# ParsaEsmati/SEA

Measured on AMD Instinct MI355X. Metric: rollout steps/sec (full-context forward, recompute mode) on cylinder_flow-shaped fields, higher is better.
Workload: dtype bf16

## Files before the change

### sea_amd/csrc/mlp_block.hip

```cpp
#include "gemm_core.hpp"
#include <stdlib.h>

struct MlpBlockLaunch {
    SeaMlpGroup g1[SEA_MAX_MLP_GROUPS];
    SeaMlp2Group g2[SEA_MAX_MLP_GROUPS];
    int tile_start[SEA_MAX_MLP_GROUPS + 1];
    int xcd_start[SEA_MAX_MLP_GROUPS + 1];
    int n_groups;
    float eps;
    int per_xcd;
    int probe;
};

__device__ __forceinline__ void glds16_blk(const void* gsrc, unsigned lds_addr) {
    unsigned keep;
    asm volatile("s_mov_b32 %0, m0\n\ts_mov_b32 m0, %2\n\ts_nop 0\n\tglobal_load_lds_dwordx4 %1, off\n\ts_mov_b32 m0, %0"
                 : "=&s"(keep) : "v"(gsrc), "s"(lds_addr) : "memory");
}

__device__ __forceinline__ void glds16_blk_s(const void* ubase, unsigned lane_off, unsigned lds_addr) {
    unsigned keep;
    asm volatile("s_mov_b32 %0, m0\n\ts_mov_b32 m0, %3\n\ts_nop 0\n\tglobal_load_lds_dwordx4 %1, %2\n\ts_mov_b32 m0, %0"
                 : "=&s"(keep) : "v"(lane_off), "s"(ubase), "s"(lds_addr) : "memory");
}

template <int KT, int NSB>
struct MlpBlockCfg {
    static constexpr int BM = 32, BKB = 128, NS = 4, NW = 8;
    static constexpr int E = KT * 64, S = NSB * 128;
    static constexpr int A_BYTES = KT * BM * BKB, STAGE = KT * 64 * BKB;
    static constexpr int PRM_OFF = A_BYTES + NS * STAGE;
    static constexpr int P1_BYTES = PRM_OFF + 2 * S * 4;
    static constexpr int SLAB_PITCH = 128 * 4 + 16, SLAB = BM * SLAB_PITCH;
    static constexpr int X3_OFF = NW * SLAB;
    static constexpr int RED2_OFF = X3_OFF + KT * BM * BKB;
    static constexpr int P2_BYTES = RED2_OFF + 2 * NW * BM * 4;
    static constexpr int RS = KT == 4 ? 8 : 4, SLOT = 16 * 128;
    static constexpr int RING_OFF = KT == 4 ? A_BYTES : P1_BYTES;
    static constexpr int RING_END = RING_OFF + NW * RS * SLOT;
    static constexpr int BYTES_ = P1_BYTES > P2_BYTES ? P1_BYTES : P2_BYTES;
    static constexpr int BYTES = BYTES_ > RING_END ? BYTES_ : RING_END;
};

__device__ __forceinline__ f32x4 mma16_first(const uint4& a, const uint4& b) {
    return __builtin_amdgcn_mfma_f32_16x16x32_bf16(__builtin_bit_cast(bf16x8, a), __builtin_bit_cast(bf16x8, b), f32x4{0.f, 0.f, 0.f, 0.f}, 0, 0, 0);
}

__device__ __forceinline__ constexpr int blk_col_base(int t, int half, int wq) { return (t >> 1) * 512 + half * 256 + wq * 64 + (t & 1) * 32; }

template <int KT, int NSB>
__global__ __launch_bounds__(512) void mlp_block_kernel(const MlpBlockLaunch L) {
    using T = __bf16;
    using Cf = MlpBlockCfg<KT, NSB>;
    constexpr int BM = 32, BKB = 128, BK = 64, NS = 4, NW = 8;
    constexpr int E = Cf::E, S = Cf::S, NSTAGE = S / 64, NT = NSB / 2;
    constexpr int A_BYTES = Cf::A_BYTES, STAGE = Cf::STAGE;
    constexpr int LPS = KT * 8 / NW;
    constexpr int PRM_OFF = Cf::PRM_OFF;
    constexpr int B1_OFF = 0, RED_OFF = S * 4;
    static_assert(RED_OFF + 2 * NW * BM * 4 <= A_BYTES && (S / 256) * 1024 <= A_BYTES && LPS * NW == KT * 8 && NT % 2 == 0 && Cf::BYTES <= 160 * 1024, "LDS layout of sea_mlp_block");
    static_assert((NT / 2) * 512 == S, "blk_col_base covers the hidden columns once");
    extern __shared__ __attribute__((aligned(16))) char smem[];
    int tile, gi = 0;
    if (L.per_xcd < 0) {
        const int xcd = (int)(blockIdx.x & 7), idx = (int)(blockIdx.x >> 3);
        if (xcd >= L.xcd_start[L.n_groups]) return;
        while (gi + 1 < L.n_groups && xcd >= L.xcd_start[gi + 1]) ++gi;
        tile = L.tile_start[gi] + (xcd - L.xcd_start[gi]) * 32 + idx;
        if (tile >= L.tile_start[gi + 1]) return;
    } else {
        tile = L.per_xcd > 0 ? (int)(blockIdx.x & 7) * L.per_xcd + (int)(blockIdx.x >> 3) : (int)blockIdx.x;
        if (tile >= L.tile_start[L.n_groups]) return;
        while (gi + 1 < L.n_groups && tile >= L.tile_start[gi + 1]) ++gi;
    }
    const SeaMlpGroup& G = L.g1[gi];
    const SeaMlp2Group& H = L.g2[gi];
    const int m0 = (tile - L.tile_start[gi]) * BM, M = G.M;
    const int tid = threadIdx.x, lane = tid & 63;
    const int wave = __builtin_amdgcn_readfirstlane(tid >> 6);
    const int r = lane & 15, g = lane >> 4;
    const int half = wave >> 2, wq = wave & 3;
    const T* A = static_cast<const T*>(G.A);
    const T* W = static_cast<const T*>(G.W1);
    const unsigned lds_base = __builtin_amdgcn_readfirstlane((unsigned)(uintptr_t)smem);
    const int rl = lane >> 3;
    const int chunk = (lane & 7) ^ (rl & 7);
    for (int p = wave; p < 2 * (S / 256); p += NW) {
        const float* src = p < S / 256 ? G.lnw : G.lnb;
        const int q = p < S / 256 ? p : p - S / 256;
        glds16_blk(src + q * 256 + lane * 4, lds_base + (unsigned)(PRM_OFF + p * 1024));
    }
    for (int p = wave; G.X32 == nullptr && p < KT * (BM / 8); p += NW) {
        const int kt = p / (BM / 8), u = p - kt * (BM / 8);
        int row = m0 + u * 8 + rl;
        row = row < M ? row : M - 1;
        glds16_blk(A + (int64_t)row * G.lda + kt * BK + chunk * 8, lds_base + (unsigned)(kt * BM * BKB + u * 8 * BKB));
    }
    const unsigned w1_lane = (unsigned)(((8 * (rl >> 2) + (rl & 3)) * G.ldw + chunk * 8) * 2);
    auto dma_stage = [&](int s) {
        const unsigned base = lds_base + (unsigned)(A_BYTES + (s % NS) * STAGE);
        const int t = s >> 2, u = (s >> 1) & 1, hs = s & 1;
#pragma unroll
        for (int i = 0; i < LPS; ++i) {
            const int p = i * NW + wave;
            const int kt = p >> 3, u8 = p & 7;
            const int urow = blk_col_base(t, hs, u8 >> 1) + 16 * (u8 & 1) + 4 * u;
            glds16_blk_s(W + (int64_t)urow * G.ldw + kt * BK, w1_lane, base + (unsigned)(kt * 64 * BKB + u8 * 8 * BKB));
        }
    };
    dma_stage(0);
    if (G.X32 != nullptr) {
        constexpr int CPT = E / 16;
        const int prow = tid >> 4, pl = tid & 15;
        int row = m0 + prow;
        row = row < M ? row : M - 1;
        const int c0 = pl * CPT;
        float xv[CPT];
#pragma unroll
        for (int c = 0; c < CPT; c += 4) load4(G.X32 + (int64_t)row * G.ldx32 + c0 + c, *reinterpret_cast<float(*)[4]>(xv + c));
        if (G.addend != nullptr) {
#pragma unroll
            for (int c = 0; c < CPT; c += 4) {
                float av[4];
                load4(G.addend + (int64_t)row * G.ldadd + c0 + c, av);
#pragma unroll
                for (int e = 0; e < 4; ++e) xv[c + e] += av[e];
            }
        }
        float gq[CPT], bq[CPT];
#pragma unroll
        for (int c = 0; c < CPT; c += 4) {
            load4(G.gamma + c0 + c, *reinterpret_cast<float(*)[4]>(gq + c));
#pragma unroll
            for (int e = 0; e < 4; ++e) bq[c + e] = 0.f;
            if (G.beta != nullptr) load4(G.beta + c0 + c, *reinterpret_cast<float(*)[4]>(bq + c));
            if (G.mod != nullptr) {
                float mw[4], mb[4];
                const T* mod = static_cast<const T*>(G.mod) + (int64_t)row * G.ldmod;
                load4(mod + c0 + c, mw);
                load4(mod + E + c0 + c, mb);
#pragma unroll
                for (int e = 0; e < 4; ++e) {
                    gq[c + e] += 1.0f + mw[e];
                    bq[c + e] += mb[e];
                }
            }
        }
        float s4[4] = {0.f, 0.f, 0.f, 0.f};
#pragma unroll
        for (int c = 0; c < CPT; c += 4)
#pragma unroll
            for (int e = 0; e < 4; ++e) s4[e] = add1(s4[e], xv[c + e]);
        float sm_ = add1(add1(s4[0], s4[1]), add1(s4[2], s4[3]));
#pragma unroll
        for (int o = 8; o >= 1; o >>= 1) sm_ += __shfl_xor(sm_, o);
        const float mean = sm_ * (1.0f / (float)E);
        float q4[4] = {0.f, 0.f, 0.f, 0.f};
#pragma unroll
        for (int c = 0; c < CPT; c += 4)
#pragma unroll
            for (int e = 0; e < 4; ++e) {
                const float d_ = xv[c + e] - mean;
                q4[e] = fma1(d_, d_, q4[e]);
            }
        float sq = add1(add1(q4[0], q4[1]), add1(q4[2], q4[3]));
#pragma unroll
        for (int o = 8; o >= 1; o >>= 1) sq += __shfl_xor(sq, o);
        const float rstd = 1.0f / sqrtf(sq * (1.0f / (float)E) + G.norm_eps);
#pragma unroll
        for (int c = 0; c < CPT; c += 8) {
            const int col = c0 + c, kt = col >> 6, ck = (col & 63) >> 3;
            bf16x8 pv;
#pragma unroll
            for (int e = 0; e < 8; ++e) pv[e] = (__bf16)((xv[c + e] - mean) * rstd * gq[c + e] + bq[c + e]);
            *reinterpret_cast<bf16x8*>(smem + kt * BM * BKB + prow * BKB + ((ck ^ (prow & 7)) << 4)) = pv;
        }
        asm volatile("s_waitcnt vmcnt(0) lgkmcnt(0)" ::: "memory");
    }
    for (int s = 1; s < NS - 1; ++s) dma_stage(s);

    const T* W2 = static_cast<const T*>(H.W2);
    const unsigned w2_lane = (unsigned)((rl * H.ldw2 + chunk * 8) * 2);
    const T* Wp = static_cast<const T*>(H.Wproj);
    const unsigned wp_lane = (unsigned)((rl * H.ldwp + chunk * 8) * 2);
    constexpr int NSLOT = (E / 16) * (NT / 2);
    constexpr int NJ = E / NW / 16;
    constexpr int NX = NJ * KT;
    auto w2_slot = [&](int k) {
        const unsigned dst = lds_base + (unsigned)(Cf::RING_OFF + (wave * Cf::RS + (k % Cf::RS)) * Cf::SLOT);
        if (k < NSLOT) {
            const int tau = k / (E / 16), j = k - tau * (E / 16);
            const T* ub = W2 + (int64_t)(j * 16) * H.ldw2 + blk_col_base(2 * tau, half, wq);
#pragma unroll
            for (int u = 0; u < 2; ++u)
                glds16_blk_s(ub + (int64_t)(8 * u) * H.ldw2, w2_lane, dst + (unsigned)(u * 1024));
        } else {
            const int kk = k - NSLOT, j = kk / KT, kt = kk - j * KT;
            const T* ub = Wp + (int64_t)(wave * (E / NW) + j * 16) * H.ldwp + kt * BK;
#pragma unroll
            for (int u = 0; u < 2; ++u)
                glds16_blk_s(ub + (int64_t)(8 * u) * H.ldwp, wp_lane, dst + (unsigned)(u * 1024));
        }
    };
    uint4 hid[NT][2];
    float mean[2], rstd[2];
    {
        f32x4 acc[NSB][2];
        uint4 areg[KT][2][2];
#pragma unroll
        for (int i = 0; i < NSB; ++i) {
            acc[i][0] = f32x4{0.f, 0.f, 0.f, 0.f};
            acc[i][1] = f32x4{0.f, 0.f, 0.f, 0.f};
        }
#pragma unroll
        for (int s = 0; s < NSTAGE; ++s) {
            if (s + 2 < NSTAGE) asm volatile("s_waitcnt vmcnt(%0) lgkmcnt(0)" ::"n"(2 * LPS) : "memory");
            else if (s + 1 < NSTAGE) asm volatile("s_waitcnt vmcnt(%0) lgkmcnt(0)" ::"n"(LPS) : "memory");
            else asm volatile("s_waitcnt vmcnt(0) lgkmcnt(0)" ::: "memory");
            __builtin_amdgcn_s_barrier();
            if (s + NS - 1 < NSTAGE) dma_stage(s + NS - 1);
            if (s == 0) {
                const char* sA = smem + r * BKB;
#pragma unroll
                for (int kt = 0; kt < KT; ++kt)
#pragma unroll
                    for (int kc = 0; kc < 2; ++kc) {
                        const int off = ((kc * 4 + g) ^ (r & 7)) << 4;
                        areg[kt][kc][0] = *reinterpret_cast<const uint4*>(sA + kt * BM * BKB + off);
                        areg[kt][kc][1] = *reinterpret_cast<const uint4*>(sA + kt * BM * BKB + 16 * BKB + off);
                    }
                asm volatile("s_waitcnt lgkmcnt(0)" ::: "memory");
            }
            if (s == 1)
                for (int p = wave; p < S / 256; p += NW) glds16_blk(G.b1 + p * 256 + lane * 4, lds_base + (unsigned)(B1_OFF + p * 1024));
            if ((s & 1) == half) {
                const char* sW = smem + A_BYTES + (s % NS) * STAGE + (wq * 16 + r) * BKB;
#pragma unroll
                for (int kt = 0; kt < KT; ++kt)
#pragma unroll
                    for (int kc = 0; kc < 2; ++kc) {
                        const int off = ((kc * 4 + g) ^ (r & 7)) << 4;
                        const uint4 wf = *reinterpret_cast<const uint4*>(sW + kt * 64 * BKB + off);
                        mma16<T>(wf, areg[kt][kc][0], acc[s >> 1][0]);
                        mma16<T>(wf, areg[kt][kc][1], acc[s >> 1][1]);
                    }
            }
        }
        if (L.probe == 1) return;
        float* red = reinterpret_cast<float*>(smem + RED_OFF);
        const float* pb1 = reinterpret_cast<const float*>(smem + B1_OFF);
        const float* pgm = reinterpret_cast<const float*>(smem + PRM_OFF);
        const float* pbt = pgm + S;
        const float inv_s = 1.0f / (float)S;
        float sum[2] = {0.f, 0.f};
#pragma unroll
        for (int i = 0; i < NSB; ++i) {
            const int n = blk_col_base(i >> 1, half, wq) + 8 * g + 4 * (i & 1);
            float bv[4];
            load4(pb1 + n, bv);
#pragma unroll
            for (int mb = 0; mb < 2; ++mb) {
#pragma unroll
                for (int q = 0; q < 4; ++q) acc[i][mb][q] += bv[q];
                sum[mb] += (acc[i][mb][0] + acc[i][mb][1]) + (acc[i][mb][2] + acc[i][mb][3]);
            }
        }
#pragma unroll
        for (int mb = 0; mb < 2; ++mb) {
            sum[mb] += __shfl_xor(sum[mb], 16);
            sum[mb] += __shfl_xor(sum[mb], 32);
            if (g == 0) red[wave * 32 + mb * 16 + r] = sum[mb];
        }
        __syncthreads();
#pragma unroll
        for (int k = 0; k < Cf::RS - 1; ++k) w2_slot(k);
        float sq[2] = {0.f, 0.f};
#pragma unroll
        for (int mb = 0; mb < 2; ++mb) {
            float t = 0.f;
#pragma unroll
            for (int w = 0; w < NW; ++w) t += red[w * 32 + mb * 16 + r];
            mean[mb] = t * inv_s;
        }
#pragma unroll
        for (int i = 0; i < NSB; ++i)
#pragma unroll
            for (int mb = 0; mb < 2; ++mb)
#pragma unroll
                for (int q = 0; q < 4; ++q) {
                    const float c = acc[i][mb][q] - mean[mb];
                    sq[mb] += c * c;
                }
#pragma unroll
        for (int mb = 0; mb < 2; ++mb) {
            sq[mb] += __shfl_xor(sq[mb], 16);
            sq[mb] += __shfl_xor(sq[mb], 32);
            if (g == 0) red[256 + wave * 32 + mb * 16 + r] = sq[mb];
        }
        asm volatile("s_waitcnt lgkmcnt(0)" ::: "memory");
        __builtin_amdgcn_s_barrier();
#pragma unroll
        for (int mb = 0; mb < 2; ++mb) {
            float t = 0.f;
#pragma unroll
            for (int w = 0; w < NW; ++w) t += red[256 + w * 32 + mb * 16 + r];
            rstd[mb] = 1.0f / sqrtf(t * inv_s + L.eps);
        }
#pragma unroll
        for (int i = 0; i < NSB; ++i) {
            const int n = blk_col_base(i >> 1, half, wq) + 8 * g + 4 * (i & 1);
            float gm[4], bt[4];
            load4(pgm + n, gm);
            load4(pbt + n, bt);
#pragma unroll
            for (int mb = 0; mb < 2; ++mb) {
                bf16x4 y;
#pragma unroll
                for (int q = 0; q < 4; ++q) y[q] = (__bf16)gelu_erf_bf16((acc[i][mb][q] - mean[mb]) * rstd[mb] * gm[q] + bt[q]);
                uint2 y2 = *reinterpret_cast<const uint2*>(&y);
                asm volatile("" : "+v"(y2.x), "+v"(y2.y));
                if (i & 1) {
                    hid[i >> 1][mb].z = y2.x;
                    hid[i >> 1][mb].w = y2.y;
                } else {
                    hid[i >> 1][mb].x = y2.x;
                    hid[i >> 1][mb].y = y2.y;
                }
            }
            __builtin_amdgcn_sched_barrier(0);
        }
    }
    __builtin_amdgcn_sched_barrier(0);
    if (L.probe == 2) {
        asm volatile("s_waitcnt vmcnt(0)" ::: "memory");
        return;
    }

    constexpr int NJB = E / 16;
    constexpr int NTOT = NSLOT + NX;
    f32x4 acc2[2][NJB];
    uint4 wp[KT * 2][NJ];
#pragma unroll
    for (int k = 0; k < NTOT; ++k) {
        const int tau = k / NJB, j = k - tau * NJB;
        {
            constexpr int AFTER_MAX = Cf::RS - 2;
            const int after = NTOT - 1 - k < AFTER_MAX ? NTOT - 1 - k : AFTER_MAX;
            switch (after) {
                case 6: asm volatile("s_waitcnt vmcnt(12) lgkmcnt(0)" ::: "memory"); break;
                case 5: asm volatile("s_waitcnt vmcnt(10) lgkmcnt(0)" ::: "memory"); break;
                case 4: asm volatile("s_waitcnt vmcnt(8) lgkmcnt(0)" ::: "memory"); break;
                case 3: asm volatile("s_waitcnt vmcnt(6) lgkmcnt(0)" ::: "memory"); break;
                case 2: asm volatile("s_waitcnt vmcnt(4) lgkmcnt(0)" ::: "memory"); break;
                case 1: asm volatile("s_waitcnt vmcnt(2) lgkmcnt(0)" ::: "memory"); break;
                default: asm volatile("s_waitcnt vmcnt(0) lgkmcnt(0)" ::: "memory"); break;
            }
        }
        if (k + Cf::RS - 1 < NTOT) w2_slot(k + Cf::RS - 1);
        const char* sl = smem + Cf::RING_OFF + (wave * Cf::RS + (k % Cf::RS)) * Cf::SLOT + r * 128;
        if (k >= NSLOT) {
            const int kk = k - NSLOT, jp = kk / KT, kt = kk - jp * KT;
#pragma unroll
            for (int kc = 0; kc < 2; ++kc) wp[kt * 2 + kc][jp] = *reinterpret_cast<const uint4*>(sl + (((kc * 4 + g) ^ (r & 7)) << 4));
            continue;
        }
#pragma unroll
        for (int u2 = 0; u2 < 2; ++u2) {
            const uint4 w = *reinterpret_cast<const uint4*>(sl + (((u2 * 4 + g) ^ (r & 7)) << 4));
            const int t = 2 * tau + u2;
            if (t == 0) {
                acc2[0][j] = mma16_first(w, hid[0][0]);
                acc2[1][j] = mma16_first(w, hid[0][1]);
            } else {
                mma16<T>(w, hid[t][0], acc2[0][j]);
                mma16<T>(w, hid[t][1], acc2[1][j]);
            }
        }
        __builtin_amdgcn_sched_barrier(0);
    }
    __syncthreads();
    if (L.probe == 3) return;
    {
    int tid_l = threadIdx.x;
    asm volatile("" : "+v"(tid_l));
    const int tid = tid_l, lane = tid & 63, r = lane & 15, g = lane >> 4;
    (void)lane;
    constexpr int NH = E / 128, JH = 8;
    const int srow = tid >> 4, scb = (tid & 15) * 8;
    float resv[NH][8];
    {
        int row = m0 + srow;
        row = row < M ? row : M - 1;
#pragma unroll
        for (int h = 0; h < NH; ++h) {
            const int col = h * 128 + scb;
            float b2a[4], b2b[4];
            load4(H.b2 + col, b2a);
            load4(H.b2 + col + 4, b2b);
            float ra[4], rb[4];
            if (H.R != nullptr) {
                load4(H.R + (int64_t)row * H.ldr + col, ra);
                load4(H.R + (int64_t)row * H.ldr + col + 4, rb);
            } else {
                load4(G.X32 + (int64_t)row * G.ldx32 + col, ra);
                load4(G.X32 + (int64_t)row * G.ldx32 + col + 4, rb);
                if (G.addend != nullptr) {
                    float aa[4], ab[4];
                    load4(G.addend + (int64_t)row * G.ldadd + col, aa);
                    load4(G.addend + (int64_t)row * G.ldadd + col + 4, ab);
#pragma unroll
                    for (int q = 0; q < 4; ++q) {
                        ra[q] += aa[q];
                        rb[q] += ab[q];
                    }
                }
            }
#pragma unroll
            for (int q = 0; q < 4; ++q) {
                resv[h][q] = b2a[q] + ra[q];
                resv[h][4 + q] = b2b[q] + rb[q];
            }
        }
    }
    constexpr int CPT = E / 16;
    const int ec0 = (tid & 15) * CPT;
    float ebp[CPT], egq[CPT], ebq[CPT];
    const bool has_norm = H.gamma != nullptr;
#pragma unroll
    for (int h = 0; h < NH; ++h) {
        char* slab = smem + wave * Cf::SLAB;
#pragma unroll
        for (int mb = 0; mb < 2; ++mb)
#pragma unroll
            for (int j = 0; j < JH; ++j)
                *reinterpret_cast<f32x4*>(slab + (mb * 16 + r) * Cf::SLAB_PITCH + (j * 16 + g * 4) * 4) = acc2[mb][h * JH + j];
        if (h == NH - 1) {
            __builtin_amdgcn_sched_barrier(0);
            int m = m0 + srow;
            m = m < M ? m : M - 1;
#pragma unroll
            for (int c = 0; c < CPT; c += 4) {
                load4(H.bproj + ec0 + c, *reinterpret_cast<float(*)[4]>(ebp + c));
#pragma unroll
                for (int q = 0; q < 4; ++q) egq[c + q] = ebq[c + q] = 0.f;
                if (has_norm) {
                    load4(H.gamma + ec0 + c, *reinterpret_cast<float(*)[4]>(egq + c));
                    if (H.beta != nullptr) load4(H.beta + ec0 + c, *reinterpret_cast<float(*)[4]>(ebq + c));
                    if (H.mod != nullptr) {
                        float mw[4], mb[4];
                        const T* mod = static_cast<const T*>(H.mod) + (int64_t)m * H.ldmod;
                        load4(mod + ec0 + c, mw);
                        load4(mod + E + ec0 + c, mb);
#pragma unroll
                        for (int q = 0; q < 4; ++q) {
                            egq[c + q] += 1.0f + mw[q];
                            ebq[c + q] += mb[q];
                        }
                    }
                }
            }
        }
        asm volatile("s_waitcnt lgkmcnt(0)" ::: "memory");
        __builtin_amdgcn_s_barrier();
        {
            float v[8];
#pragma unroll
            for (int q = 0; q < 8; ++q) v[q] = resv[h][q];
#pragma unroll
            for (int w = 0; w < NW; ++w) {
                const float4 a = *reinterpret_cast<const float4*>(smem + w * Cf::SLAB + srow * Cf::SLAB_PITCH + scb * 4);
                const float4 b = *reinterpret_cast<const float4*>(smem + w * Cf::SLAB + srow * Cf::SLAB_PITCH + scb * 4 + 16);
                v[0] += a.x; v[1] += a.y; v[2] += a.z; v[3] += a.w;
                v[4] += b.x; v[5] += b.y; v[6] += b.z; v[7] += b.w;
            }
            const int col = h * 128 + scb, kt = col >> 6, ck = (col & 63) >> 3;
            bf16x8 pv;
#pragma unroll
            for (int q = 0; q < 8; ++q) pv[q] = (__bf16)v[q];
            *reinterpret_cast<bf16x8*>(smem + Cf::X3_OFF + kt * BM * BKB + srow * BKB + ((ck ^ (srow & 7)) << 4)) = pv;
        }
        asm volatile("s_waitcnt lgkmcnt(0)" ::: "memory");
        __builtin_amdgcn_s_barrier();
        if (L.probe == 5 + h) return;
    }

    if (L.probe == 4) return;
    f32x4 acc3[2][NJ];
    {
        const char* sA = smem + Cf::X3_OFF + r * BKB;
#pragma unroll
        for (int kt = 0; kt < KT; ++kt)
#pragma unroll
            for (int kc = 0; kc < 2; ++kc) {
                const int off = ((kc * 4 + g) ^ (r & 7)) << 4;
                const uint4 af0 = *reinterpret_cast<const uint4*>(sA + kt * BM * BKB + off);
                const uint4 af1 = *reinterpret_cast<const uint4*>(sA + kt * BM * BKB + 16 * BKB + off);
#pragma unroll
                for (int j = 0; j < NJ; ++j) {
                    if (kt == 0 && kc == 0) {
                        acc3[0][j] = mma16_first(wp[0][j], af0);
                        acc3[1][j] = mma16_first(wp[0][j], af1);
                    } else {
                        mma16<T>(wp[kt * 2 + kc][j], af0, acc3[0][j]);
                        mma16<T>(wp[kt * 2 + kc][j], af1, acc3[1][j]);
                    }
                }
            }
    }
    constexpr int SEG = 80, YP = (E / 16) * SEG + 16;
    static_assert(BM * YP <= Cf::X3_OFF, "the y tile lies in front of the x3 tile");
#pragma unroll
    for (int i = 0; i < 2; ++i)
#pragma unroll
        for (int j = 0; j < NJ; ++j) {
            const int n = wave * (E / NW) + j * 16 + g * 4;
            *reinterpret_cast<f32x4*>(smem + (i * 16 + r) * YP + (n >> 4) * SEG + (n & 15) * 4) = acc3[i][j];
        }
    asm volatile("s_waitcnt lgkmcnt(0)" ::: "memory");
    __builtin_amdgcn_s_barrier();
    {
        float v[CPT];
#pragma unroll
        for (int c = 0; c < CPT; c += 4) {
            const float4 y = *reinterpret_cast<const float4*>(smem + srow * YP + ((ec0 + c) >> 4) * SEG + ((ec0 + c) & 15) * 4);
            v[c] = y.x + ebp[c]; v[c + 1] = y.y + ebp[c + 1]; v[c + 2] = y.z + ebp[c + 2]; v[c + 3] = y.w + ebp[c + 3];
        }
        if (has_norm) {
            float s4[4] = {0.f, 0.f, 0.f, 0.f};
#pragma unroll
            for (int c = 0; c < CPT; c += 4)
#pragma unroll
                for (int e = 0; e < 4; ++e) s4[e] = add1(s4[e], v[c + e]);
            float sm_ = add1(add1(s4[0], s4[1]), add1(s4[2], s4[3]));
#pragma unroll
            for (int o = 8; o >= 1; o >>= 1) sm_ += __shfl_xor(sm_, o);
            const float mean2 = sm_ * (1.0f / (float)E);
            float q4[4] = {0.f, 0.f, 0.f, 0.f};
#pragma unroll
            for (int c = 0; c < CPT; c += 4)
#pragma unroll
                for (int e = 0; e < 4; ++e) {
                    const float d_ = v[c + e] - mean2;
                    q4[e] = fma1(d_, d_, q4[e]);
                }
            float sq = add1(add1(q4[0], q4[1]), add1(q4[2], q4[3]));
#pragma unroll
            for (int o = 8; o >= 1; o >>= 1) sq += __shfl_xor(sq, o);
            const float rstd2 = 1.0f / sqrtf(sq * (1.0f / (float)E) + L.eps);
#pragma unroll
            for (int c = 0; c < CPT; ++c) v[c] = (v[c] - mean2) * rstd2 * egq[c] + ebq[c];
        }
        const int m = m0 + srow;
        if (m < M) {
#pragma unroll
            for (int c = 0; c < CPT; c += 4) {
                if (H.Y32 != nullptr) store4(H.Y32 + (int64_t)m * H.ldy32 + ec0 + c, v[c], v[c + 1], v[c + 2], v[c + 3]);
                if (H.Yact != nullptr) store4(static_cast<T*>(H.Yact) + (int64_t)m * H.ldyact + ec0 + c, v[c], v[c + 1], v[c + 2], v[c + 3]);
            }
        }
    }
    }
}

extern "C" int sea_mlp_block(const SeaMlpGroup* g1, const SeaMlp2Group* g2, int n_groups, float eps, int dtype, void* stream) {
    SEA_REQUIRE(g1 != nullptr && g2 != nullptr && n_groups >= 1 && n_groups <= SEA_MAX_MLP_GROUPS, "sea_mlp_block: n_groups=%d out of range", n_groups);
    const int E = g1[0].E, S = g1[0].S;
    const bool shape_ok = (E == 256 && S == 2048) || (E == 128 && S == 1024);
    if (dtype != SEA_BF16 || !shape_ok) {
        sea_set_error("sea_mlp_block: unsupported dtype / shape (dtype=%d E=%d S=%d): bf16, (E, S) in {(256, 2048), (128, 1024)}", dtype, E, S);
        return SEA_EUNSUPPORTED;
    }
    MlpBlockLaunch L;
    memset(&L, 0, sizeof(L));
    int total = 0;
    for (int i = 0; i < n_groups; ++i) {
        const SeaMlpGroup& G = g1[i];
        const SeaMlp2Group& H = g2[i];
        SEA_REQUIRE(G.E == E && G.S == S && H.E == E && H.S == S && G.M >= 1 && H.M == G.M, "sea_mlp_block[%d]: the groups of a launch share E and S; both halves the same M", i);
        SEA_REQUIRE((G.A || G.X32) && G.W1 && G.b1 && G.lnw && G.lnb, "sea_mlp_block[%d]: null pointer (first layer)", i);
        SEA_REQUIRE((G.X32 || (G.lda % 8 == 0 && G.lda >= E)) && G.ldw % 8 == 0 && G.ldw >= E, "sea_mlp_block[%d]: bad strides (first layer)", i);
        if (G.X32 != nullptr)
            SEA_REQUIRE(G.gamma && G.ldx32 % 4 == 0 && G.ldx32 >= E && (!G.addend || (G.ldadd % 4 == 0 && G.ldadd >= E)) && G.Xout == nullptr &&
                            (!G.mod || (G.ldmod % 8 == 0 && G.ldmod >= 2 * E)) && sea_aligned16(G.X32) && sea_aligned16(G.addend) && sea_aligned16(G.mod) &&
                            sea_aligned16(G.gamma) && sea_aligned16(G.beta) && G.norm_eps > 0.f,
                        "sea_mlp_block[%d]: norm prologue: null / misaligned pointer, bad stride, or Xout (the block keeps x + addend to itself)", i);
        SEA_REQUIRE(sea_aligned16(G.A) && sea_aligned16(G.W1) && sea_aligned16(G.b1) && sea_aligned16(G.lnw) && sea_aligned16(G.lnb), "sea_mlp_block[%d]: pointers must be 16-byte aligned", i);
        SEA_REQUIRE(H.W2 && H.b2 && (H.R || G.X32) && H.Wproj && H.bproj && (H.Y32 || H.Yact), "sea_mlp_block[%d]: null pointer (second layer; R may be NULL with the norm prologue: the residual is then x + addend)", i);
        SEA_REQUIRE(H.ldw2 % 8 == 0 && H.ldw2 >= S && H.ldwp % 8 == 0 && H.ldwp >= E && (!H.R || (H.ldr % 4 == 0 && H.ldr >= E)) &&
                        (!H.Y32 || (H.ldy32 % 4 == 0 && H.ldy32 >= E)) && (!H.Yact || (H.ldyact % 4 == 0 && H.ldyact >= E)) && (!H.mod || (H.ldmod % 4 == 0 && H.ldmod >= 2 * E)),
                    "sea_mlp_block[%d]: bad strides (second layer)", i);
        SEA_REQUIRE(sea_aligned16(H.W2) && sea_aligned16(H.b2) && sea_aligned16(H.R) && sea_aligned16(H.Wproj) && sea_aligned16(H.bproj) && sea_aligned16(H.gamma) && sea_aligned16(H.beta) &&
                        sea_aligned16(H.mod) && sea_aligned16(H.Y32) && sea_aligned16(H.Yact),
                    "sea_mlp_block[%d]: pointers must be 16-byte aligned", i);
        SEA_REQUIRE(H.gamma || (!H.beta && !H.mod), "sea_mlp_block[%d]: beta / mod without gamma", i);
        L.g1[i] = G;
        L.g2[i] = H;
        L.tile_start[i] = total;
        total += (G.M + 31) / 32;
    }
    L.tile_start[n_groups] = total;
    L.n_groups = n_groups;
    L.eps = eps;
    static const int probe = sea_tune("blk_probe", 0);
    L.probe = probe;
    hipStream_t s = static_cast<hipStream_t>(stream);
    int xcds = 0;
    for (int i = 0; i < n_groups; ++i) {
        L.xcd_start[i] = xcds;
        xcds += (L.tile_start[i + 1] - L.tile_start[i] + 31) / 32;
    }
    L.xcd_start[n_groups] = xcds;
    static const int xcd_excl = sea_tune("blk_xcd", 0);
    static const int per_xcd_on = sea_tune("blk_perxcd", 1);
    if (total > 256 && per_xcd_on) {
        L.per_xcd = (total + 7) / 8;
        total = 8 * L.per_xcd;
    } else if (xcds <= 8 && xcd_excl) {
        L.per_xcd = -1;
        total = 256;
    }
    if (E == 256) {
        constexpr int lds = MlpBlockCfg<4, 16>::BYTES;
        static const hipError_t once = hipFuncSetAttribute(reinterpret_cast<const void*>(mlp_block_kernel<4, 16>), hipFuncAttributeMaxDynamicSharedMemorySize, lds);
        (void)once;
        mlp_block_kernel<4, 16><<<dim3(total), dim3(512), lds, s>>>(L);
    } else {
        constexpr int lds = MlpBlockCfg<2, 8>::BYTES;
        static const hipError_t once = hipFuncSetAttribute(reinterpret_cast<const void*>(mlp_block_kernel<2, 8>), hipFuncAttributeMaxDynamicSharedMemorySize, lds);
        (void)once;
        mlp_block_kernel<2, 8><<<dim3(total), dim3(512), lds, s>>>(L);
    }
    SEA_CHECK_LAUNCH("sea_mlp_block");
    return SEA_OK;
}
```

Before: 5201.

## Stream W1 through per-wave LDS rings instead of block-wide staged pipeline

```diff
diff --git a/sea_amd/csrc/mlp_block.hip b/sea_amd/csrc/mlp_block.hip
--- a/sea_amd/csrc/mlp_block.hip
+++ b/sea_amd/csrc/mlp_block.hip
@@ -26,21 +26,39 @@
 
 template <int KT, int NSB>
 struct MlpBlockCfg {
-    static constexpr int BM = 32, BKB = 128, NS = 4, NW = 8;
+    static constexpr int BM = 32, BKB = 128, NW = 8;
     static constexpr int E = KT * 64, S = NSB * 128;
-    static constexpr int A_BYTES = KT * BM * BKB, STAGE = KT * 64 * BKB;
-    static constexpr int PRM_OFF = A_BYTES + NS * STAGE;
+    static constexpr int A_BYTES = KT * BM * BKB;
+    static constexpr int RS = KT == 4 ? 8 : 4, SLOT = 16 * 128;
+    static constexpr int RING_OFF = A_BYTES;
+    static constexpr int PRM_OFF = RING_OFF + NW * RS * SLOT;
     static constexpr int P1_BYTES = PRM_OFF + 2 * S * 4;
     static constexpr int SLAB_PITCH = 128 * 4 + 16, SLAB = BM * SLAB_PITCH;
     static constexpr int X3_OFF = NW * SLAB;
     static constexpr int RED2_OFF = X3_OFF + KT * BM * BKB;
     static constexpr int P2_BYTES = RED2_OFF + 2 * NW * BM * 4;
-    static constexpr int RS = KT == 4 ? 8 : 4, SLOT = 16 * 128;
-    static constexpr int RING_OFF = KT == 4 ? A_BYTES : P1_BYTES;
-    static constexpr int RING_END = RING_OFF + NW * RS * SLOT;
-    static constexpr int BYTES_ = P1_BYTES > P2_BYTES ? P1_BYTES : P2_BYTES;
-    static constexpr int BYTES = BYTES_ > RING_END ? BYTES_ : RING_END;
+    static constexpr int BYTES = P1_BYTES > P2_BYTES ? P1_BYTES : P2_BYTES;
 };
+
+__device__ __forceinline__ void ring_wait(int n) {
+    switch (n) {
+        case 14: asm volatile("s_waitcnt vmcnt(14) lgkmcnt(0)" ::: "memory"); break;
+        case 13: asm volatile("s_waitcnt vmcnt(13) lgkmcnt(0)" ::: "memory"); break;
+        case 12: asm volatile("s_waitcnt vmcnt(12) lgkmcnt(0)" ::: "memory"); break;
+        case 11: asm volatile("s_waitcnt vmcnt(11) lgkmcnt(0)" ::: "memory"); break;
+        case 10: asm volatile("s_waitcnt vmcnt(10) lgkmcnt(0)" ::: "memory"); break;
+        case 9: asm volatile("s_waitcnt vmcnt(9) lgkmcnt(0)" ::: "memory"); break;
+        case 8: asm volatile("s_waitcnt vmcnt(8) lgkmcnt(0)" ::: "memory"); break;
+        case 7: asm volatile("s_waitcnt vmcnt(7) lgkmcnt(0)" ::: "memory"); break;
+        case 6: asm volatile("s_waitcnt vmcnt(6) lgkmcnt(0)" ::: "memory"); break;
+        case 5: asm volatile("s_waitcnt vmcnt(5) lgkmcnt(0)" ::: "memory"); break;
+        case 4: asm volatile("s_waitcnt vmcnt(4) lgkmcnt(0)" ::: "memory"); break;
+        case 3: asm volatile("s_waitcnt vmcnt(3) lgkmcnt(0)" ::: "memory"); break;
+        case 2: asm volatile("s_waitcnt vmcnt(2) lgkmcnt(0)" ::: "memory"); break;
+        case 1: asm volatile("s_waitcnt vmcnt(1) lgkmcnt(0)" ::: "memory"); break;
+        default: asm volatile("s_waitcnt vmcnt(0) lgkmcnt(0)" ::: "memory"); break;
+    }
+}
 
 __device__ __forceinline__ f32x4 mma16_first(const uint4& a, const uint4& b) {
     return __builtin_amdgcn_mfma_f32_16x16x32_bf16(__builtin_bit_cast(bf16x8, a), __builtin_bit_cast(bf16x8, b), f32x4{0.f, 0.f, 0.f, 0.f}, 0, 0, 0);
@@ -52,13 +70,13 @@
 __global__ __launch_bounds__(512) void mlp_block_kernel(const MlpBlockLaunch L) {
     using T = __bf16;
     using Cf = MlpBlockCfg<KT, NSB>;
-    constexpr int BM = 32, BKB = 128, BK = 64, NS = 4, NW = 8;
-    constexpr int E = Cf::E, S = Cf::S, NSTAGE = S / 64, NT = NSB / 2;
-    constexpr int A_BYTES = Cf::A_BYTES, STAGE = Cf::STAGE;
-    constexpr int LPS = KT * 8 / NW;
+    constexpr int BM = 32, BKB = 128, BK = 64, NW = 8;
+    constexpr int E = Cf::E, S = Cf::S, NT = NSB / 2;
+    constexpr int A_BYTES = Cf::A_BYTES;
     constexpr int PRM_OFF = Cf::PRM_OFF;
     constexpr int B1_OFF = 0, RED_OFF = S * 4;
-    static_assert(RED_OFF + 2 * NW * BM * 4 <= A_BYTES && (S / 256) * 1024 <= A_BYTES && LPS * NW == KT * 8 && NT % 2 == 0 && Cf::BYTES <= 160 * 1024, "LDS layout of sea_mlp_block");
+    static_assert(RED_OFF + 2 * NW * BM * 4 <= A_BYTES && (S / 256) * 1024 <= A_BYTES && S / 256 <= NW && NT % 2 == 0 && Cf::BYTES <= 160 * 1024, "LDS layout of sea_mlp_block");
+    static_assert(2 * (Cf::RS - 1) <= 14, "ring_wait names every count of the rings");
     static_assert((NT / 2) * 512 == S, "blk_col_base covers the hidden columns once");
     extern __shared__ __attribute__((aligned(16))) char smem[];
     int tile, gi = 0;
@@ -97,18 +115,16 @@
         glds16_blk(A + (int64_t)row * G.lda + kt * BK + chunk * 8, lds_base + (unsigned)(kt * BM * BKB + u * 8 * BKB));
     }
     const unsigned w1_lane = (unsigned)(((8 * (rl >> 2) + (rl & 3)) * G.ldw + chunk * 8) * 2);
-    auto dma_stage = [&](int s) {
-        const unsigned base = lds_base + (unsigned)(A_BYTES + (s % NS) * STAGE);
-        const int t = s >> 2, u = (s >> 1) & 1, hs = s & 1;
-#pragma unroll
-        for (int i = 0; i < LPS; ++i) {
-            const int p = i * NW + wave;
-            const int kt = p >> 3, u8 = p & 7;
-            const int urow = blk_col_base(t, hs, u8 >> 1) + 16 * (u8 & 1) + 4 * u;
-            glds16_blk_s(W + (int64_t)urow * G.ldw + kt * BK, w1_lane, base + (unsigned)(kt * 64 * BKB + u8 * 8 * BKB));
-        }
+    const T* W1w = W + (int64_t)blk_col_base(0, half, wq) * G.ldw;
+    constexpr int NK1 = NSB * KT;
+    auto w1_slot = [&](int k) {
+        const unsigned dst = lds_base + (unsigned)(Cf::RING_OFF + (wave * Cf::RS + (k % Cf::RS)) * Cf::SLOT);
+        const int i = k / KT, kt = k - i * KT;
+        const T* ub = W1w + (int64_t)(blk_col_base(i >> 1, 0, 0) + 4 * (i & 1)) * G.ldw + kt * BK;
+#pragma unroll
+        for (int u8 = 0; u8 < 2; ++u8)
+            glds16_blk_s(ub + (int64_t)(16 * u8) * G.ldw, w1_lane, dst + (unsigned)(u8 * 1024));
     };
-    dma_stage(0);
     if (G.X32 != nullptr) {
         constexpr int CPT = E / 16;
         const int prow = tid >> 4, pl = tid & 15;
@@ -177,7 +193,8 @@
         }
         asm volatile("s_waitcnt vmcnt(0) lgkmcnt(0)" ::: "memory");
     }
-    for (int s = 1; s < NS - 1; ++s) dma_stage(s);
+#pragma unroll
+    for (int k = 0; k < Cf::RS - 1; ++k) w1_slot(k);
 
     const T* W2 = static_cast<const T*>(H.W2);
     const unsigned w2_lane = (unsigned)((rl * H.ldw2 + chunk * 8) * 2);
@@ -207,46 +224,52 @@
     {
         f32x4 acc[NSB][2];
         uint4 areg[KT][2][2];
-#pragma unroll
-        for (int i = 0; i < NSB; ++i) {
-            acc[i][0] = f32x4{0.f, 0.f, 0.f, 0.f};
-            acc[i][1] = f32x4{0.f, 0.f, 0.f, 0.f};
-        }
-#pragma unroll
-        for (int s = 0; s < NSTAGE; ++s) {
-            if (s + 2 < NSTAGE) asm volatile("s_waitcnt vmcnt(%0) lgkmcnt(0)" ::"n"(2 * LPS) : "memory");
-            else if (s + 1 < NSTAGE) asm volatile("s_waitcnt vmcnt(%0) lgkmcnt(0)" ::"n"(LPS) : "memory");
-            else asm volatile("s_waitcnt vmcnt(0) lgkmcnt(0)" ::: "memory");
-            __builtin_amdgcn_s_barrier();
-            if (s + NS - 1 < NSTAGE) dma_stage(s + NS - 1);
-            if (s == 0) {
-                const char* sA = smem + r * BKB;
-#pragma unroll
-                for (int kt = 0; kt < KT; ++kt)
-#pragma unroll
-                    for (int kc = 0; kc < 2; ++kc) {
-                        const int off = ((kc * 4 + g) ^ (r & 7)) << 4;
-                        areg[kt][kc][0] = *reinterpret_cast<const uint4*>(sA + kt * BM * BKB + off);
-                        areg[kt][kc][1] = *reinterpret_cast<const uint4*>(sA + kt * BM * BKB + 16 * BKB + off);
-                    }
-                asm volatile("s_waitcnt lgkmcnt(0)" ::: "memory");
-            }
-            if (s == 1)
-                for (int p = wave; p < S / 256; p += NW) glds16_blk(G.b1 + p * 256 + lane * 4, lds_base + (unsigned)(B1_OFF + p * 1024));
-            if ((s & 1) == half) {
-                const char* sW = smem + A_BYTES + (s % NS) * STAGE + (wq * 16 + r) * BKB;
-#pragma unroll
-                for (int kt = 0; kt < KT; ++kt)
-#pragma unroll
-                    for (int kc = 0; kc < 2; ++kc) {
-                        const int off = ((kc * 4 + g) ^ (r & 7)) << 4;
-                        const uint4 wf = *reinterpret_cast<const uint4*>(sW + kt * 64 * BKB + off);
-                        mma16<T>(wf, areg[kt][kc][0], acc[s >> 1][0]);
-                        mma16<T>(wf, areg[kt][kc][1], acc[s >> 1][1]);
-                    }
-            }
+        ring_wait(2 * (Cf::RS - 1));
+        __builtin_amdgcn_s_barrier();
+        {
+            const char* sA = smem + r * BKB;
+#pragma unroll
+            for (int kt = 0; kt < KT; ++kt)
+#pragma unroll
+                for (int kc = 0; kc < 2; ++kc) {
+                    const int off = ((kc * 4 + g) ^ (r & 7)) << 4;
+                    areg[kt][kc][0] = *reinterpret_cast<const uint4*>(sA + kt * BM * BKB + off);
+                    areg[kt][kc][1] = *reinterpret_cast<const uint4*>(sA + kt * BM * BKB + 16 * BKB + off);
+                }
+        }
+        asm volatile("s_waitcnt lgkmcnt(0)" ::: "memory");
+        __builtin_amdgcn_s_barrier();
+        if (L.probe == 9) {
+            asm volatile("s_waitcnt vmcnt(0)" ::: "memory");
+            return;
+        }
+        for (int p = wave; p < S / 256; p += NW) glds16_blk(G.b1 + p * 256 + lane * 4, lds_base + (unsigned)(B1_OFF + p * 1024));
+        constexpr int B1P = S / 256 == NW ? 1 : 0;
+#pragma unroll
+        for (int k = 0; k < NK1; ++k) {
+            const int after = NK1 - 1 - k < Cf::RS - 2 ? NK1 - 1 - k : Cf::RS - 2;
+            ring_wait(2 * after + (k <= Cf::RS - 2 ? B1P : 0));
+            if (k + Cf::RS - 1 < NK1) w1_slot(k + Cf::RS - 1);
+            const char* sl = smem + Cf::RING_OFF + (wave * Cf::RS + (k % Cf::RS)) * Cf::SLOT + r * 128;
+            const int i = k / KT, kt = k - i * KT;
+#pragma unroll
+            for (int kc = 0; kc < 2; ++kc) {
+                const uint4 wf = *reinterpret_cast<const uint4*>(sl + (((kc * 4 + g) ^ (r & 7)) << 4));
+                if (kt == 0 && kc == 0) {
+                    acc[i][0] = mma16_first(wf, areg[0][0][0]);
+                    acc[i][1] = mma16_first(wf, areg[0][0][1]);
+                } else {
+                    mma16<T>(wf, areg[kt][kc][0], acc[i][0]);
+                    mma16<T>(wf, areg[kt][kc][1], acc[i][1]);
+                }
+            }
+            __builtin_amdgcn_sched_barrier(0);
         }
         if (L.probe == 1) return;
+        asm volatile("s_waitcnt lgkmcnt(0)" ::: "memory");
+#pragma unroll
+        for (int k = 0; k < Cf::RS - 1; ++k) w2_slot(k);
+        __builtin_amdgcn_s_barrier();
         float* red = reinterpret_cast<float*>(smem + RED_OFF);
         const float* pb1 = reinterpret_cast<const float*>(smem + B1_OFF);
         const float* pgm = reinterpret_cast<const float*>(smem + PRM_OFF);
@@ -271,9 +294,8 @@
             sum[mb] += __shfl_xor(sum[mb], 32);
             if (g == 0) red[wave * 32 + mb * 16 + r] = sum[mb];
         }
-        __syncthreads();
-#pragma unroll
-        for (int k = 0; k < Cf::RS - 1; ++k) w2_slot(k);
+        asm volatile("s_waitcnt lgkmcnt(0)" ::: "memory");
+        __builtin_amdgcn_s_barrier();
         float sq[2] = {0.f, 0.f};
 #pragma unroll
         for (int mb = 0; mb < 2; ++mb) {
@@ -343,19 +365,7 @@
 #pragma unroll
     for (int k = 0; k < NTOT; ++k) {
         const int tau = k / NJB, j = k - tau * NJB;
-        {
-            constexpr int AFTER_MAX = Cf::RS - 2;
-            const int after = NTOT - 1 - k < AFTER_MAX ? NTOT - 1 - k : AFTER_MAX;
-            switch (after) {
-                case 6: asm volatile("s_waitcnt vmcnt(12) lgkmcnt(0)" ::: "memory"); break;
-                case 5: asm volatile("s_waitcnt vmcnt(10) lgkmcnt(0)" ::: "memory"); break;
-                case 4: asm volatile("s_waitcnt vmcnt(8) lgkmcnt(0)" ::: "memory"); break;
-                case 3: asm volatile("s_waitcnt vmcnt(6) lgkmcnt(0)" ::: "memory"); break;
-                case 2: asm volatile("s_waitcnt vmcnt(4) lgkmcnt(0)" ::: "memory"); break;
-                case 1: asm volatile("s_waitcnt vmcnt(2) lgkmcnt(0)" ::: "memory"); break;
-                default: asm volatile("s_waitcnt vmcnt(0) lgkmcnt(0)" ::: "memory"); break;
-            }
-        }
+        ring_wait(2 * (NTOT - 1 - k < Cf::RS - 2 ? NTOT - 1 - k : Cf::RS - 2));
         if (k + Cf::RS - 1 < NTOT) w2_slot(k + Cf::RS - 1);
         const char* sl = smem + Cf::RING_OFF + (wave * Cf::RS + (k % Cf::RS)) * Cf::SLOT + r * 128;
         if (k >= NSLOT) {
```

New measurement: 5254 (median of 6 runs). +1.0%, better.
